# liuzhenboo/Stereo-Visual-Odometry

Measured on AMD Instinct MI355X. Metric: stereo frames/sec on KITTI-00 1241x376; LK-kernel achieved HBM GB/s vs peak, higher is better.
Workload: dtype u8; 1 GPU; S0 synthetic KITTI-like stereo sequence 1241x376 (config #2 stand-in), FAST+LK track_mode LK_stereof2f_pnp, batched frame pairs (256 per step, 4 distinct chunks cycled), frames resident in HBM for `value`; `m1` (--full) = host-resident frames, H2D included; pairs_ok_last_step=256, parallelism=1 GPU

## Files before the change

### include/svo_abi.h

```cpp
#ifndef SVO_ABI_H
#define SVO_ABI_H

#include <stdint.h>

#ifdef __cplusplus
extern "C" {
#endif

#define SVO_ABI_VERSION 9

#define SVO_OK                 0
#define SVO_ERR_ARG           -1
#define SVO_ERR_HIP           -2
#define SVO_ERR_NOMEM         -3
#define SVO_ERR_STATE         -4
#define SVO_FAIL_FEW_KEYPOINTS 1
#define SVO_FAIL_FEW_TRACKS    2
#define SVO_FAIL_INLIER_RATIO  3
#define SVO_FAIL_ROTATION_GATE 4
#define SVO_FAIL_TRANSL_GATE   5
#define SVO_FAIL_CAPACITY      6

#define SVO_MEM_HOST   0
#define SVO_MEM_DEVICE 1

typedef struct svo_ctx svo_ctx;

typedef struct { float x, y; } svo_pt2f;
typedef struct { float x, y, z; } svo_pt3f;
typedef struct {
    float x, y, size, angle, response;
    int32_t octave, class_id;
} svo_keypoint;

typedef struct {
    int32_t width, height;
    int32_t max_keypoints;
    int32_t max_batch;
    int32_t num_slots;
    int32_t fast_threshold;
    int32_t num_features_tracking;
    int32_t iterations;
    float   reproj_err;
    float   confidence;
    double  feature_match_error;
    double  inlier_rate;
    double  min_move2, max_move2;
    double  P1[12], P2[12];
    int32_t track_mode;
    int32_t orb_nfeatures;
    float   orb_scale_factor;
    int32_t orb_nlevels;
    int32_t orb_ini_th, orb_min_th;
    int32_t lk_accum;
    int32_t fast_keep_strongest;
} svo_config;

#define SVO_MODE_LK  0
#define SVO_MODE_ORB 1
#define SVO_LK_ACCUM_EXACT 0
#define SVO_LK_ACCUM_SSE2  1
#define SVO_LK_ACCUM_SIMD128 2
#define SVO_LK_ACCUM_SSE2_LEGACY 3

typedef struct {
    double rvec[3], tvec[3], R[9];
    int32_t n_inliers, ransac_iters, best_iter, lm_iters, ok, _pad;
} svo_pnp_result;

typedef struct {
    int32_t ok;
    int32_t fail_stage;
    int32_t n_prev_kps, n_cur_kps, n_tracked, n_inliers;
    int32_t ransac_iters, lm_iters;
    double  rvec[3], tvec[3], R[9];
    double  T_rel_inv[16];
    double  pose[16];
} svo_step_result;

int         svo_abi_version(void);
int         svo_config_bytes(void);
void        svo_default_config(svo_config *cfg, int width, int height);
int         svo_device_count(int *n);
int         svo_create(const svo_config *cfg, int device, svo_ctx **out);
void        svo_destroy(svo_ctx *ctx);
const char *svo_last_error(const svo_ctx *ctx);
int         svo_set_stream(svo_ctx *ctx, void *hip_stream);
int         svo_sync(svo_ctx *ctx);
int         svo_wait_stream(svo_ctx *ctx, void *hip_stream);
int         svo_signal_stream(svo_ctx *ctx, void *hip_stream);
int         svo_signal_stream_inputs(svo_ctx *ctx, void *hip_stream);
int         svo_num_levels(const svo_ctx *ctx);


int svo_fast_detect(svo_ctx *ctx, const uint8_t *img, int pitch, int mem, int threshold,
                    int nonmax, svo_keypoint *out, int cap, int *n_out);

int svo_build_pyramid(svo_ctx *ctx, int slot, const uint8_t *img, int pitch, int mem);
int svo_read_pyramid_level(svo_ctx *ctx, int slot, int level, uint8_t *out, int out_pitch, int mem,
                           int *w, int *h);

int svo_lk_track(svo_ctx *ctx, int slot_prev, int slot_next, const svo_pt2f *prev_pts, int n,
                 svo_pt2f *next_pts, uint8_t *status, int mem);

int svo_circular_match(svo_ctx *ctx, int slot_prevL, int slot_prevR, int slot_curL, int slot_curR,
                       const svo_pt2f *t1_left, int n, svo_pt2f *out_t1_left,
                       svo_pt2f *out_t1_right, svo_pt2f *out_t2_right, svo_pt2f *out_t2_left,
                       int *m_out, int mem);

int svo_triangulate(svo_ctx *ctx, const double P1[12], const double P2[12], const svo_pt2f *x1,
                    const svo_pt2f *x2, int n, svo_pt3f *out, int mem);

int svo_pnp_ransac(svo_ctx *ctx, const svo_pt3f *obj, const svo_pt2f *img, int n, const double K[9],
                   int iterations, float reproj_err, double confidence, svo_pnp_result *res,
                   uint8_t *inlier_mask, int mem);

int svo_orb_extract(svo_ctx *ctx, const uint8_t *img, int pitch, int mem, svo_keypoint *kps, uint8_t *desc,
                    int cap, int *n_out, int *per_level);
int svo_orb_read_level(svo_ctx *ctx, int level, uint8_t *out, int *w, int *h);
int svo_orb_read_candidates(svo_ctx *ctx, int level, float *out4, int cap, int *n_out);

int svo_match_hamming(svo_ctx *ctx, const uint8_t *query, int nq, const uint8_t *train, int nt, int32_t *train_idx,
                      float *distance, int mem);


int svo_add_frame(svo_ctx *ctx, const uint8_t *left, const uint8_t *right, int pitch, int mem,
                  svo_step_result *res);
int svo_reset(svo_ctx *ctx);
int svo_get_pose(svo_ctx *ctx, double pose[16]);
int svo_set_pose(svo_ctx *ctx, const double pose[16]);

int svo_track_batch(svo_ctx *ctx, const uint8_t *left_frames, const uint8_t *right_frames,
                    int pitch, int64_t frame_stride, int n_frames, const double *pose0,
                    svo_step_result *results, int results_mem);

int svo_set_overlap(svo_ctx *ctx, int on);
int svo_wait_results(svo_ctx *ctx);

int svo_host_alloc(svo_ctx *ctx, size_t bytes, void **out);
int svo_host_free(svo_ctx *ctx, void *p);
int svo_upload_frames(svo_ctx *ctx, int buf, const uint8_t *left_frames, const uint8_t *right_frames,
                      int pitch, int64_t frame_stride, int n_frames);
int svo_upload_frames_at(svo_ctx *ctx, int buf, int first_slot, const uint8_t *left_frames, const uint8_t *right_frames,
                         int pitch, int64_t frame_stride, int n_frames);
int svo_wait_upload(svo_ctx *ctx, int buf);
int svo_track_uploaded(svo_ctx *ctx, int buf, int n_frames, const double *pose0,
                       svo_step_result *results, int results_mem);
#define SVO_CONTINUE_CHAIN       1
#define SVO_CONTINUE_CARRY_FRAME 2
int svo_track_uploaded_async(svo_ctx *ctx, int buf, int n_frames, const double *pose0, int continue_chain);
int svo_collect_results(svo_ctx *ctx, svo_step_result *results, int n_pairs);
int svo_results_ready(svo_ctx *ctx, int *n_pairs);

int svo_get_frame_keypoints(svo_ctx *ctx, int side, svo_keypoint *kps, uint8_t *descriptors, int cap, int *n_out);
int svo_get_last_tracks(svo_ctx *ctx, svo_pt2f *t1_left, svo_pt2f *t1_right, svo_pt2f *t2_right,
                        svo_pt2f *t2_left, uint8_t *inlier, int cap, int *n_out);
int svo_get_batch_tracks(svo_ctx *ctx, int pair, svo_pt2f *t1_left, svo_pt2f *t1_right, svo_pt2f *t2_right,
                         svo_pt2f *t2_left, uint8_t *inlier, int cap, int *n_out);

int svo_streams_create(svo_ctx *ctx, int n_streams);
int svo_streams_count(const svo_ctx *ctx, int *n_streams);
int svo_streams_step(svo_ctx *ctx, const int32_t *stream_ids, int m, const uint8_t *left_frames,
                     const uint8_t *right_frames, int pitch, int64_t frame_stride, int mem,
                     svo_step_result *results, int results_mem);
int svo_streams_reset(svo_ctx *ctx, int stream_id);
int svo_streams_get_pose(svo_ctx *ctx, int stream_id, double pose[16]);
int svo_streams_set_pose(svo_ctx *ctx, int stream_id, const double pose[16]);
int svo_streams_get_tracks(svo_ctx *ctx, int item, svo_pt2f *t1_left, svo_pt2f *t1_right, svo_pt2f *t2_right,
                           svo_pt2f *t2_left, uint8_t *inlier, int cap, int *n_out);

#define SVO_INTERP_NEAREST 0
#define SVO_INTERP_LINEAR  1
int svo_scale_projection(const double P[12], double inv_x, double inv_y, int interp, double P_out[12]);
int svo_resize(svo_ctx *ctx, const uint8_t *src, int sw, int sh, int spitch, int64_t sstride,
               uint8_t *dst, int dw, int dh, int dpitch, int64_t dstride, int n_frames,
               int interp, double fx, double fy, int mem);
int svo_ingest_create(svo_ctx *ctx, int src_width, int src_height, int interp, double fx, double fy);
int svo_ingest_info(const svo_ctx *ctx, int *src_width, int *src_height, int *interp, double *inv_x, double *inv_y);
int svo_ingest_add_frame(svo_ctx *ctx, const uint8_t *left, const uint8_t *right, int pitch, int mem, svo_step_result *res);
int svo_ingest_track_batch(svo_ctx *ctx, const uint8_t *lefts, const uint8_t *rights, int pitch, int64_t frame_stride,
                           int n_frames, const double *pose0, svo_step_result *results, int results_mem);
int svo_ingest_streams_step(svo_ctx *ctx, const int32_t *stream_ids, int m, const uint8_t *lefts, const uint8_t *rights,
                            int pitch, int64_t frame_stride, int mem, svo_step_result *results, int results_mem);
// ... 57 lines not shown
```

### stereo-visual-odometry_amd/binding.py

```python
import ctypes as C
import os
import subprocess

import numpy as np

_HERE = os.path.dirname(os.path.abspath(__file__))
_LIB = None

MEM_HOST, MEM_DEVICE = 0, 1

KP_DTYPE = np.dtype([("x", "<f4"), ("y", "<f4"), ("size", "<f4"), ("angle", "<f4"),
                     ("response", "<f4"), ("octave", "<i4"), ("class_id", "<i4")])


class SvoError(RuntimeError):
    pass


class Config(C.Structure):
    _fields_ = [("width", C.c_int32), ("height", C.c_int32), ("max_keypoints", C.c_int32),
                ("max_batch", C.c_int32), ("num_slots", C.c_int32), ("fast_threshold", C.c_int32),
                ("num_features_tracking", C.c_int32), ("iterations", C.c_int32),
                ("reproj_err", C.c_float), ("confidence", C.c_float),
                ("feature_match_error", C.c_double), ("inlier_rate", C.c_double),
# ... 57 lines not shown
    return library_path()


def load_library():
    global _LIB
    if _LIB is not None:
        return _LIB
    path = library_path()
    if not os.path.exists(path):
        raise SvoError(f"{path} is missing: run __graft_entry__.build() (hipcc) first; "
                       "this package has no CPU fallback")
    lib = C.CDLL(path)
    if lib.svo_config_bytes() != C.sizeof(Config):
        raise SvoError(f"{path}: svo_config is {lib.svo_config_bytes()} bytes, this binding's Config {C.sizeof(Config)} "
                       "(stale build? run __graft_entry__.build())")
    lib.svo_last_error.restype = C.c_char_p
    lib.svo_last_error.argtypes = [C.c_void_p]
    lib.svo_create.argtypes = [C.POINTER(Config), C.c_int, C.POINTER(C.c_void_p)]
    lib.svo_destroy.argtypes = [C.c_void_p]
    lib.svo_destroy.restype = None
    lib.svo_default_config.argtypes = [C.POINTER(Config), C.c_int, C.c_int]
    lib.svo_default_config.restype = None
    lib.svo_track_batch.argtypes = [C.c_void_p, C.c_void_p, C.c_void_p, C.c_int, C.c_int64, C.c_int,
                                    C.c_void_p, C.c_void_p, C.c_int]
    lib.svo_get_frame_keypoints.argtypes = [C.c_void_p, C.c_int, C.c_void_p, C.c_void_p, C.c_int, C.POINTER(C.c_int)]
    lib.svo_get_last_tracks.argtypes = [C.c_void_p] + [C.c_void_p] * 5 + [C.c_int, C.POINTER(C.c_int)]
    lib.svo_get_batch_tracks.argtypes = [C.c_void_p, C.c_int] + [C.c_void_p] * 5 + [C.c_int, C.POINTER(C.c_int)]
    lib.svo_chain_relative.argtypes = [C.c_void_p, C.c_void_p, C.c_void_p, C.c_int, C.c_void_p, C.c_void_p, C.c_int]
    lib.svo_host_alloc.argtypes = [C.c_void_p, C.c_size_t, C.POINTER(C.c_void_p)]
    lib.svo_host_free.argtypes = [C.c_void_p, C.c_void_p]
    lib.svo_upload_frames.argtypes = [C.c_void_p, C.c_int, C.c_void_p, C.c_void_p, C.c_int, C.c_int64, C.c_int]
    lib.svo_upload_frames_at.argtypes = [C.c_void_p, C.c_int, C.c_int, C.c_void_p, C.c_void_p, C.c_int, C.c_int64, C.c_int]
    lib.svo_wait_stream.argtypes = [C.c_void_p, C.c_void_p]
    lib.svo_signal_stream.argtypes = [C.c_void_p, C.c_void_p]
    lib.svo_signal_stream_inputs.argtypes = [C.c_void_p, C.c_void_p]
    lib.svo_wait_upload.argtypes = [C.c_void_p, C.c_int]
    lib.svo_track_uploaded.argtypes = [C.c_void_p, C.c_int, C.c_int, C.c_void_p, C.c_void_p, C.c_int]
    lib.svo_track_uploaded_async.argtypes = [C.c_void_p, C.c_int, C.c_int, C.c_void_p, C.c_int]
    lib.svo_collect_results.argtypes = [C.c_void_p, C.c_void_p, C.c_int]
    lib.svo_results_ready.argtypes = [C.c_void_p, C.POINTER(C.c_int)]
    lib.svo_set_pose.argtypes = [C.c_void_p, C.c_void_p]
    lib.svo_streams_create.argtypes = [C.c_void_p, C.c_int]
    lib.svo_streams_count.argtypes = [C.c_void_p, C.POINTER(C.c_int)]
    lib.svo_streams_step.argtypes = [C.c_void_p, C.c_void_p, C.c_int, C.c_void_p, C.c_void_p, C.c_int, C.c_int64, C.c_int,
                                     C.c_void_p, C.c_int]
    lib.svo_streams_reset.argtypes = [C.c_void_p, C.c_int]
    lib.svo_streams_get_pose.argtypes = [C.c_void_p, C.c_int, C.c_void_p]
    lib.svo_streams_set_pose.argtypes = [C.c_void_p, C.c_int, C.c_void_p]
    lib.svo_streams_get_tracks.argtypes = [C.c_void_p, C.c_int] + [C.c_void_p] * 5 + [C.c_int, C.POINTER(C.c_int)]
    lib.svo_scale_projection.argtypes = [C.c_void_p, C.c_double, C.c_double, C.c_int, C.c_void_p]
    lib.svo_resize.argtypes = [C.c_void_p, C.c_void_p, C.c_int, C.c_int, C.c_int, C.c_int64,
                               C.c_void_p, C.c_int, C.c_int, C.c_int, C.c_int64, C.c_int, C.c_int, C.c_double, C.c_double, C.c_int]
    lib.svo_ingest_create.argtypes = [C.c_void_p, C.c_int, C.c_int, C.c_int, C.c_double, C.c_double]
    lib.svo_ingest_info.argtypes = [C.c_void_p, C.POINTER(C.c_int), C.POINTER(C.c_int), C.POINTER(C.c_int),
                                    C.POINTER(C.c_double), C.POINTER(C.c_double)]
    lib.svo_ingest_add_frame.argtypes = [C.c_void_p, C.c_void_p, C.c_void_p, C.c_int, C.c_int, C.c_void_p]
    lib.svo_ingest_track_batch.argtypes = lib.svo_track_batch.argtypes
    lib.svo_ingest_streams_step.argtypes = lib.svo_streams_step.argtypes
    lib.svo_ingest_upload_frames_at.argtypes = lib.svo_upload_frames_at.argtypes
    lib.svo_set_fast_buckets.argtypes = [C.c_void_p, C.c_int, C.c_int, C.c_int]
    lib.svo_get_fast_buckets.argtypes = [C.c_void_p, C.POINTER(C.c_int), C.POINTER(C.c_int), C.POINTER(C.c_int)]
    lib.svo_bucket_corners.argtypes = [C.c_void_p, C.c_void_p, C.c_int, C.c_int, C.c_int, C.c_int, C.c_int, C.c_int,
                                       C.c_void_p, C.c_int, C.c_void_p, C.c_int]
    lib.svo_set_lk_detector.argtypes = [C.c_void_p, C.c_int, C.c_int, C.c_double, C.c_double]
    lib.svo_get_lk_detector.argtypes = [C.c_void_p, C.POINTER(C.c_int), C.POINTER(C.c_int), C.POINTER(C.c_double),
                                        C.POINTER(C.c_double)]
    lib.svo_min_eigen_map.argtypes = [C.c_void_p, C.c_void_p, C.c_int, C.c_int, C.c_int, C.c_int, C.c_void_p, C.c_int]
    lib.svo_gftt_detect.argtypes = [C.c_void_p, C.c_void_p, C.c_int, C.c_int, C.c_int, C.c_int, C.c_int, C.c_double, C.c_double,
                                    C.c_void_p, C.c_void_p, C.c_int, C.c_void_p]
    lib.svo_set_pose_refine.argtypes = [C.c_void_p, C.c_int, C.c_int, C.c_int, C.c_double, C.c_int]
    lib.svo_get_pose_refine.argtypes = [C.c_void_p, C.POINTER(C.c_int), C.POINTER(C.c_int), C.POINTER(C.c_int),
                                        C.POINTER(C.c_double), C.POINTER(C.c_int)]
    lib.svo_refine_pose.argtypes = [C.c_void_p, C.c_void_p, C.c_void_p, C.c_void_p, C.c_int, C.c_void_p, C.c_void_p, C.c_void_p,
                                    C.c_void_p, C.POINTER(RefineResult), C.c_void_p, C.c_int]
    lib.svo_get_refine_result.argtypes = [C.c_void_p, C.c_int, C.POINTER(RefineResult), C.c_void_p, C.c_int, C.POINTER(C.c_int)]
    lib.svo_set_orb_matcher.argtypes = [C.c_void_p, C.c_int, C.c_int, C.c_int, C.c_double, C.c_double, C.c_double]
    lib.svo_get_orb_matcher.argtypes = [C.c_void_p, C.POINTER(C.c_int), C.POINTER(C.c_int), C.POINTER(C.c_int),
                                        C.POINTER(C.c_double), C.POINTER(C.c_double), C.POINTER(C.c_double)]
    lib.svo_orb_stereo_frame.argtypes = [C.c_void_p, C.c_void_p, C.c_void_p, C.c_int, C.c_int, C.c_int, C.c_void_p, C.c_void_p,
                                         C.c_void_p, C.c_int, C.POINTER(C.c_int)]
    lib.svo_orb_track_frames.argtypes = [C.c_void_p, C.c_int, C.c_int, C.c_void_p, C.c_void_p, C.c_void_p, C.c_void_p, C.c_void_p,
                                         C.c_int, C.POINTER(C.c_int)]
    lib.svo_get_frame_stereo.argtypes = [C.c_void_p, C.c_void_p, C.c_void_p, C.c_int, C.POINTER(C.c_int)]
    _LIB = lib
    return lib


def _interp(interp):
    if isinstance(interp, str):
        if interp not in ("nearest", "linear"):
            raise ValueError(f"interp must be 'nearest' or 'linear', not {interp!r}")
        return INTERP_LINEAR if interp == "linear" else INTERP_NEAREST
    return int(interp)


def scale_projection(P, inv_x, inv_y, interp="nearest"):
    P = np.ascontiguousarray(P, np.float64).reshape(12)
    out = np.zeros(12)
    rc = load_library().svo_scale_projection(C.c_void_p(P.ctypes.data), float(inv_x), float(inv_y), _interp(interp),
                                             C.c_void_p(out.ctypes.data))
    if rc != 0:
        raise SvoError(f"svo_scale_projection failed ({rc}): inv must be in (0, 1], interp nearest or linear")
    return out.reshape(3, 4)


def device_count():
    n = C.c_int(0)
    load_library().svo_device_count(C.byref(n))
    return n.value


def default_config(width, height, **overrides):
    cfg = Config()
    load_library().svo_default_config(C.byref(cfg), int(width), int(height))
    for k, v in overrides.items():
        if k in ("P1", "P2"):
            arr = getattr(cfg, k)
            for i, x in enumerate(np.asarray(v, np.float64).reshape(12)):
                arr[i] = float(x)
        else:
            setattr(cfg, k, v)
    return cfg


def _ptr(a):
    if a is None:
        return None, MEM_HOST
    if isinstance(a, np.ndarray):
        assert a.flags["C_CONTIGUOUS"]
        return C.c_void_p(a.ctypes.data), MEM_HOST
    assert a.is_contiguous()
    return C.c_void_p(a.data_ptr()), (MEM_DEVICE if a.is_cuda else MEM_HOST)


def _pose_ptr(pose0):
    if pose0 is None:
        return None
    return np.ascontiguousarray(pose0, np.float64).reshape(16).ctypes.data_as(C.c_void_p)


def _records(n, results):
    if results is None:
        out = np.zeros(n, dtype=STEP_DTYPE)
        return out, C.c_void_p(out.ctypes.data), MEM_HOST
    return results, C.c_void_p(results.data_ptr()), MEM_DEVICE


class Context:

    def __init__(self, width, height, device=0, **cfg_overrides):
        self.lib = load_library()
        self.cfg = default_config(width, height, **cfg_overrides)
        h = C.c_void_p()
        rc = self.lib.svo_create(C.byref(self.cfg), int(device), C.byref(h))
        if rc != 0:
            raise SvoError(f"svo_create failed with {rc} (no usable HIP device?) -- there is no CPU fallback")
        self.h = h
        self.width, self.height = int(width), int(height)

    def close(self):
        if getattr(self, "h", None):
            self.lib.svo_destroy(self.h)
            self.h = None

    def __del__(self):
        try:
# ... 5 lines not shown
        if rc < 0 or (rc > 0 and not allow_soft):
            raise SvoError(f"svo call failed ({rc}): {self.lib.svo_last_error(self.h).decode()}")
        return rc

    def sync(self):
        self._check(self.lib.svo_sync(self.h))

    def set_stream(self, stream_handle):
        self._check(self.lib.svo_set_stream(self.h, C.c_void_p(stream_handle)))
        self._stream_handle = int(stream_handle or 0)

    def wait_stream(self, stream_handle):
        self._check(self.lib.svo_wait_stream(self.h, C.c_void_p(stream_handle)))

    def signal_stream(self, stream_handle):
        self._check(self.lib.svo_signal_stream(self.h, C.c_void_p(stream_handle)))

    def signal_stream_inputs(self, stream_handle):
        self._check(self.lib.svo_signal_stream_inputs(self.h, C.c_void_p(stream_handle)))

    def _order_in(self, t):
        import torch
        other = torch.cuda.current_stream(t.device).cuda_stream
        if other and other == getattr(self, "_stream_handle", 0):
            return False
        self.wait_stream(other)
        return True

    def _order_out(self, t):
        import torch
        other = torch.cuda.current_stream(t.device).cuda_stream
        if other and other == getattr(self, "_stream_handle", 0):
            return
        self.signal_stream(other)

    @property
    def num_levels(self):
        return self.lib.svo_num_levels(self.h)

    def set_overlap(self, on=True):
        self._check(self.lib.svo_set_overlap(self.h, int(on)))

    def wait_results(self):
        self._check(self.lib.svo_wait_results(self.h))

    def enable_timing(self, on=True):
        self._check(self.lib.svo_enable_timing(self.h, int(on)))

    def get_timing(self):
        names = (C.c_char_p * 64)()
        ms = (C.c_float * 64)()
        n = self.lib.svo_get_timing(self.h, names, ms, 64)
        return [(names[i].decode(), float(ms[i])) for i in range(n)]

    def _img(self, img, shape=None):
        shape = shape or (self.height, self.width)
        assert tuple(img.shape) == tuple(shape), (tuple(img.shape), shape)
        if isinstance(img, np.ndarray):
            assert img.dtype == np.uint8 and img.strides[1] == 1
            return C.c_void_p(img.ctypes.data), int(img.strides[0]), MEM_HOST
        assert img.element_size() == 1 and img.stride(1) == 1
        return C.c_void_p(img.data_ptr()), int(img.stride(0)), (MEM_DEVICE if img.is_cuda else MEM_HOST)

    def fast_detect(self, img, threshold=20, nonmax=True, cap=None):
        cap = cap or self.cfg.max_keypoints
        p, pitch, mem = self._img(img)
        out = np.zeros(cap, dtype=KP_DTYPE)
        n = C.c_int(0)
        self._check(self.lib.svo_fast_detect(self.h, p, pitch, mem, int(threshold), int(bool(nonmax)),
                                             C.c_void_p(out.ctypes.data), cap, C.byref(n)))
        return out[:n.value].copy()

    def build_pyramid(self, slot, img):
        p, pitch, mem = self._img(img)
        self._check(self.lib.svo_build_pyramid(self.h, int(slot), p, pitch, mem))

    def read_pyramid_level(self, slot, level):
        w, h = C.c_int(0), C.c_int(0)
        self._check(self.lib.svo_read_pyramid_level(self.h, slot, level, None, 0, MEM_HOST,
                                                    C.byref(w), C.byref(h)))
        out = np.zeros((h.value, w.value), np.uint8)
        self._check(self.lib.svo_read_pyramid_level(self.h, slot, level, C.c_void_p(out.ctypes.data),
                                                    w.value, MEM_HOST, C.byref(w), C.byref(h)))
        return out

    def lk_track(self, slot_prev, slot_next, pts):
        if isinstance(pts, np.ndarray):
            pts = np.ascontiguousarray(pts, np.float32).reshape(-1, 2)
            n = pts.shape[0]
            out = np.zeros((n, 2), np.float32)
            st = np.zeros(n, np.uint8)
        else:
            import torch
            n = pts.shape[0]
            out = torch.zeros((n, 2), dtype=torch.float32, device=pts.device)
            st = torch.zeros(n, dtype=torch.uint8, device=pts.device)
            self._order_in(st)
        pi, mem = _ptr(pts)
        po, _ = _ptr(out)
        ps, _ = _ptr(st)
        self._check(self.lib.svo_lk_track(self.h, slot_prev, slot_next, pi, n, po, ps, mem))
        if mem == MEM_DEVICE:
            self._order_out(st)
        return out, st

    def circular_match(self, slots, t1_left):
        if isinstance(t1_left, np.ndarray):
            t1_left = np.ascontiguousarray(t1_left, np.float32).reshape(-1, 2)
            n = t1_left.shape[0]
            outs = [np.zeros((max(n, 1), 2), np.float32) for _ in range(4)]
        else:
            import torch
            n = t1_left.shape[0]
            outs = [torch.zeros((max(n, 1), 2), dtype=torch.float32, device=t1_left.device) for _ in range(4)]
            self._order_in(outs[0])
        pi, mem = _ptr(t1_left)
        m = C.c_int(0)
        self._check(self.lib.svo_circular_match(self.h, *[int(s) for s in slots], pi, n,
                                                *[_ptr(o)[0] for o in outs], C.byref(m), mem))
        return [o[:m.value] for o in outs]

    def triangulate(self, P1, P2, x1, x2):
        P1 = np.ascontiguousarray(P1, np.float64).reshape(12)
        P2 = np.ascontiguousarray(P2, np.float64).reshape(12)
        if isinstance(x1, np.ndarray):
            x1 = np.ascontiguousarray(x1, np.float32).reshape(-1, 2)
            x2 = np.ascontiguousarray(x2, np.float32).reshape(-1, 2)
            out = np.zeros((x1.shape[0], 3), np.float32)
        else:
            import torch
            out = torch.zeros((x1.shape[0], 3), dtype=torch.float32, device=x1.device)
            self._order_in(out)
        p1, mem = _ptr(x1)
        p2, _ = _ptr(x2)
        self._check(self.lib.svo_triangulate(self.h, C.c_void_p(P1.ctypes.data), C.c_void_p(P2.ctypes.data),
                                             p1, p2, x1.shape[0], _ptr(out)[0], mem))
        if mem == MEM_DEVICE:
            self._order_out(out)
        return out

    def pnp_ransac(self, obj, img, K, iterations=500, reproj_err=0.5, confidence=0.99):
        K = np.ascontiguousarray(K, np.float64).reshape(9)
        if isinstance(obj, np.ndarray):
            obj = np.ascontiguousarray(obj, np.float32).reshape(-1, 3)
            img = np.ascontiguousarray(img, np.float32).reshape(-1, 2)
            mask = np.zeros(max(obj.shape[0], 1), np.uint8)
        else:
            import torch
            mask = torch.zeros(max(obj.shape[0], 1), dtype=torch.uint8, device=obj.device)
            self._order_in(mask)
        n = obj.shape[0]
        res = PnPResult()
        po, mem = _ptr(obj)
        conf = float(np.float32(confidence))
        self._check(self.lib.svo_pnp_ransac(self.h, po, _ptr(img)[0], n, C.c_void_p(K.ctypes.data),
                                            int(iterations), C.c_float(reproj_err), C.c_double(conf),
                                            C.byref(res), _ptr(mask)[0], mem))
        if mem == MEM_DEVICE:
            self._order_out(mask)
            mask = mask.cpu().numpy()
        return dict(ok=res.ok, rvec=np.array(res.rvec), tvec=np.array(res.tvec),
                    R=np.array(res.R).reshape(3, 3), n_inliers=res.n_inliers,
                    ransac_iters=res.ransac_iters, best_iter=res.best_iter, lm_iters=res.lm_iters,
                    mask=np.asarray(mask[:n]).copy())

    def set_pose_refine(self, mode, rounds=4, iters=10, sigma_px=1.0, min_inliers=6):
# ... 490 lines not shown
```

### stereo-visual-odometry_amd/csrc/pyramid.hip

```cpp
#include "svo_device.h"
#include "svo_kernels.h"

namespace svo {

__device__ __forceinline__ const uint8_t *src_image(const PyrArgs &a, int b)
{
    if (a.img2) return ((b & 1) ? a.img2 : a.img) + (int64_t)(b >> 1) * a.img_stride;
    return a.img + (int64_t)b * a.img_stride;
}

__global__ __launch_bounds__(256) void pyr_copy0_kernel(PyrArgs a)
{
    const int b = blockIdx.z, y = blockIdx.y * blockDim.y + threadIdx.y;
    const int w = a.g.w[0];
    if (y >= a.g.h[0]) return;
    const uint8_t *src = src_image(a, b) + (int64_t)y * a.pitch;
    uint8_t *dst = a.slots + (int64_t)b * a.slot_stride + a.g.origin[0] + (int64_t)y * a.g.pitch[0];
    const int x = (blockIdx.x * blockDim.x + threadIdx.x) * 16;
    if (x >= w) return;
    if (x + 16 <= w && ((uintptr_t)(src + x) & 15) == 0) {
        *(uint4 *)(dst + x) = *(const uint4 *)(src + x);
    } else {
        for (int q = 0; q < 16 && x + q < w; q++) dst[x + q] = src[x + q];
    }
}

constexpr int kBorderRows = 16;
constexpr int kFrameRowsPerWg = 4, kSidePasses = 4;
__host__ __device__ inline int border_top_groups() { return 2 * kPad / kFrameRowsPerWg; }
__host__ __device__ inline int border_side_groups(int h) { return (h + kBorderRows * kSidePasses - 1) / (kBorderRows * kSidePasses); }
__global__ __launch_bounds__(256) void pyr_border_kernel(PyrArgs a, int l)
{
    const int b = blockIdx.y;
    const int w = a.g.w[l], h = a.g.h[l], pitch = a.g.pitch[l];
    uint8_t *lvl = a.slots + (int64_t)b * a.slot_stride + a.g.origin[l];
    if ((int)blockIdx.x < border_top_groups()) {
        for (int q = 0; q < kFrameRowsPerWg; q++) {
            const int gidx = blockIdx.x * kFrameRowsPerWg + q;
            const int py = gidx < kPad ? gidx - kPad : h + (gidx - kPad);
            const uint8_t *src = lvl + (int64_t)refl101(py, h) * pitch;
            uint8_t *dst = lvl + (int64_t)py * pitch;
            for (int px = ((int)threadIdx.x << 2) - kPad; px < w + kPad; px += 1024) {
                uint32_t v = 0;
                if (px >= 0 && px + 4 <= w) v = *(const uint32_t *)(src + px);
                else {
#pragma unroll
                    for (int k = 0; k < 4; k++) v |= (uint32_t)src[refl101(min(px + k, w + kPad - 1), w)] << (8 * k);
                }
                if (px + 4 <= w + kPad) *(uint32_t *)(dst + px) = v;
                else for (int k = 0; px + k < w + kPad; k++) dst[px + k] = (uint8_t)(v >> (8 * k));
            }
        }
        return;
    }
    const int sgroup = blockIdx.x - border_top_groups();
    if (w >= 2 * kPad) {
        static_assert(kBorderRows == 16 && kPad == 32, "256 threads = 16 rows x 16 dwords");
        typedef uint32_t u32_unaligned __attribute__((aligned(1)));
        const int k = threadIdx.x & 15, r = threadIdx.x >> 4;
        const int px = k < 8 ? -kPad + 4 * k : w + 4 * (k - 8);
        const int c0 = k < 8 ? kPad - 3 - 4 * k : w - 5 - 4 * (k - 8);
        for (int q = 0; q < kSidePasses; q++) {
            const int py = (sgroup * kSidePasses + q) * kBorderRows + r;
            if (py >= h) return;
            uint8_t *row = lvl + (int64_t)py * pitch;
            const uint32_t v = *(const u32_unaligned *)(row + c0);
            *(u32_unaligned *)(row + px) = __builtin_amdgcn_perm(0u, v, 0x00010203u);
        }
    } else {
        const int t = threadIdx.x & 63;
        const int px = t < kPad ? t - kPad : w + (t - kPad);
        const int sx = refl101(px, w);
        for (int q = 0; q < kSidePasses; q++)
            for (int r = threadIdx.x >> 6; r < kBorderRows; r += 4) {
                const int py = (sgroup * kSidePasses + q) * kBorderRows + r;
                if (py >= h) return;
                uint8_t *row = lvl + (int64_t)py * pitch;
                row[px] = row[sx];
            }
    }
}

__global__ __launch_bounds__(256) void pyr_down_kernel(PyrArgs a, int l)
{
    const int b = blockIdx.z, y = blockIdx.y * blockDim.y + threadIdx.y;
    const int w = a.g.w[l];
    if (y >= a.g.h[l]) return;
    const int sp = a.g.pitch[l - 1];
    uint8_t *slot = a.slots + (int64_t)b * a.slot_stride;
    const uint8_t *src = slot + a.g.origin[l - 1];
    uint8_t *dst = slot + a.g.origin[l] + (int64_t)y * a.g.pitch[l];
    const int x0 = (blockIdx.x * blockDim.x + threadIdx.x) * 4;
    if (x0 >= w) return;
    int acc[4] = {0, 0, 0, 0};
#pragma unroll
    for (int r = 0; r < 5; r++) {
        const uint32_t *row = (const uint32_t *)(src + (int64_t)(2 * y + r - 2) * sp + 2 * x0 - 4);
        const uint32_t d0 = row[0], d1 = row[1], d2 = row[2], d3 = row[3];
        int s[16];
#pragma unroll
        for (int j = 0; j < 4; j++) {
            s[j] = (d0 >> (8 * j)) & 255; s[4 + j] = (d1 >> (8 * j)) & 255;
            s[8 + j] = (d2 >> (8 * j)) & 255; s[12 + j] = (d3 >> (8 * j)) & 255;
        }
        const int wv = (r == 2) ? 6 : ((r == 1 || r == 3) ? 4 : 1);
#pragma unroll
        for (int q = 0; q < 4; q++) {
            const int c = 4 + 2 * q;
            const int hs = s[c] * 6 + (s[c - 1] + s[c + 1]) * 4 + s[c - 2] + s[c + 2];
            acc[q] += hs * wv;
        }
    }
    uint32_t out = 0;
#pragma unroll
    for (int q = 0; q < 4; q++) out |= (uint32_t)((acc[q] + 128) >> 8) << (8 * q);
    if (x0 + 4 <= w) *(uint32_t *)(dst + x0) = out;
    else for (int q = 0; x0 + q < w; q++) dst[x0 + q] = (uint8_t)(out >> (8 * q));
}

__global__ __launch_bounds__(256) void pyr_read_level_kernel(PyrGeom g, const uint8_t *slot, int l,
                                                              uint8_t *out, int out_pitch)
{
    int x = blockIdx.x * 256 + threadIdx.x, y = blockIdx.y;
    if (x >= g.w[l]) return;
    out[(int64_t)y * out_pitch + x] = slot[g.origin[l] + (int64_t)y * g.pitch[l] + x];
}

void launch_pyramid(const PyrArgs &a, int batch, hipStream_t st)
{
    dim3 blk(256, 1, 1);
    auto shape = [](int lanes_per_row, int rows, dim3 &grid, dim3 &block, int batch) {
        const int bx = lanes_per_row < 256 ? lanes_per_row : 256, by = 256 / bx;
        block = dim3(bx, by, 1);
        grid = dim3((lanes_per_row + bx - 1) / bx, (rows + by - 1) / by, batch);
    };
    {
        dim3 g, bk;
        shape((a.g.w[0] + 15) / 16, a.g.h[0], g, bk, batch);
        hipLaunchKernelGGL(pyr_copy0_kernel, g, bk, 0, st, a);
    }
    for (int l = 0; l < a.g.nlevels; l++) {
        if (l > 0) {
            dim3 g, bk;
            shape((a.g.w[l] + 3) / 4, a.g.h[l], g, bk, batch);
            hipLaunchKernelGGL(pyr_down_kernel, g, bk, 0, st, a, l);
        }
        dim3 gb(border_top_groups() + border_side_groups(a.g.h[l]), batch, 1);
        hipLaunchKernelGGL(pyr_border_kernel, gb, blk, 0, st, a, l);
    }
}

void launch_pyr_read_level(const PyrGeom &g, const uint8_t *slot, int l, uint8_t *out, int out_pitch,
                           hipStream_t st)
{
    dim3 grid((g.w[l] + 255) / 256, g.h[l], 1), blk(256, 1, 1);
    hipLaunchKernelGGL(pyr_read_level_kernel, grid, blk, 0, st, g, slot, l, out, out_pitch);
}

}
```

### stereo-visual-odometry_amd/csrc/svo_abi.hip

```cpp
#include <cmath>
#include <cstdio>
#include <cstring>
#include <ctime>
#include <new>
#include <vector>
#include "svo_ctx.h"

using namespace svo;

static int align_up(int v, int a) { return (v + a - 1) / a * a; }

namespace svo {
int dev_alloc_raw(svo_ctx *ctx, void **out, size_t bytes)
{
    *out = nullptr;
    if (bytes == 0) bytes = 1;
    if (ctx->arena.planning) {
        ctx->arena.plan.emplace_back(out, ctx->arena.planned);
        ctx->arena.planned += (bytes + 255) / 256 * 256;
        return SVO_OK;
    }
    SVO_HIP(hipMalloc(out, bytes));
    ctx->arena.extra.push_back(*out);
    return SVO_OK;
// ... 382 lines not shown
    return svo::stage_host_image(ctx, img, pitch, stage_idx, dptr, dpitch);
}

extern "C" int svo_fast_detect(svo_ctx *ctx, const uint8_t *img, int pitch, int mem, int threshold,
                               int nonmax, svo_keypoint *out, int cap, int *n_out)
{
    if (!ctx) return SVO_ERR_ARG;
    SVO_ARG(out && n_out && cap >= 0, "null output");
    SVO_HIP(hipSetDevice(ctx->device));
    const uint8_t *d; int dp;
    int rc = resolve_image(ctx, img, pitch, mem, 0, &d, &dp);
    if (rc) return rc;
    FastArgs a{};
    a.img = d; a.pitch = dp; a.img_stride = 0;
    a.w = ctx->cfg.width; a.h = ctx->cfg.height;
    a.thr = threshold < 0 ? 0 : (threshold > 255 ? 255 : threshold);
    a.nms = nonmax != 0;
    a.score = ctx->score; a.spitch = ctx->spitch; a.score_stride = ctx->score_stride;
    a.rowcount = ctx->rowcount; a.rowcount_stride = ctx->rowcount_stride;
    a.kp_xy = ctx->kp_xy; a.kp_resp = ctx->kp_resp; a.kp_stride = ctx->cfg.max_keypoints;
    a.n_out = ctx->kp_n; a.cap = ctx->cfg.max_keypoints;
    launch_fast(a, 1, ctx->stream);
    SVO_HIP(hipGetLastError());
    int *h_n = (int *)ctx->h_pinned;
    SVO_HIP(hipMemcpyAsync(h_n, ctx->kp_n, sizeof(int), hipMemcpyDeviceToHost, ctx->stream));
    SVO_HIP(hipStreamSynchronize(ctx->stream));
    int n = *h_n;
    *n_out = n;
    if (n > ctx->cfg.max_keypoints) { ctx->err = "FAST: keypoints exceed max_keypoints"; return SVO_ERR_ARG; }
    if (n > cap) { ctx->err = "FAST: keypoints exceed caller capacity"; return SVO_ERR_ARG; }
    if (n == 0) return SVO_OK;
    float2 *h_xy = (float2 *)((char *)ctx->h_pinned + 256);
    float *h_r = (float *)(h_xy + ctx->cfg.max_keypoints);
    SVO_HIP(hipMemcpyAsync(h_xy, ctx->kp_xy, sizeof(float2) * n, hipMemcpyDeviceToHost, ctx->stream));
    SVO_HIP(hipMemcpyAsync(h_r, ctx->kp_resp, sizeof(float) * n, hipMemcpyDeviceToHost, ctx->stream));
    SVO_HIP(hipStreamSynchronize(ctx->stream));
    for (int i = 0; i < n; i++) {
        out[i].x = h_xy[i].x; out[i].y = h_xy[i].y; out[i].size = 7.f; out[i].angle = -1.f;
        out[i].response = h_r[i]; out[i].octave = 0; out[i].class_id = -1;
    }
    return SVO_OK;
}

extern "C" int svo_build_pyramid(svo_ctx *ctx, int slot, const uint8_t *img, int pitch, int mem)
{
    if (!ctx) return SVO_ERR_ARG;
    SVO_ARG(slot >= 0 && slot < ctx->cfg.num_slots, "slot out of range");
    SVO_HIP(hipSetDevice(ctx->device));
    const uint8_t *d; int dp;
    int rc = resolve_image(ctx, img, pitch, mem, 0, &d, &dp);
    if (rc) return rc;
    PyrArgs a{};
    a.g = ctx->geom; a.img = d; a.pitch = dp; a.img_stride = 0;
    a.slots = ctx->slots + (size_t)slot * ctx->geom.slot_bytes; a.slot_stride = 0;
    launch_pyramid(a, 1, ctx->stream);
    SVO_HIP(hipGetLastError());
    if (mem == SVO_MEM_HOST) SVO_HIP(hipStreamSynchronize(ctx->stream));
    ctx->slot_built[slot] = 1;
    return SVO_OK;
}

extern "C" int svo_read_pyramid_level(svo_ctx *ctx, int slot, int level, uint8_t *out, int out_pitch,
                                      int mem, int *w, int *h)
{
    if (!ctx) return SVO_ERR_ARG;
    SVO_ARG(slot >= 0 && slot < ctx->cfg.num_slots, "slot out of range");
    SVO_ARG(level >= 0 && level < ctx->geom.nlevels, "level out of range");
    if (!ctx->slot_built[slot]) { ctx->err = "pyramid slot not built"; return SVO_ERR_STATE; }
    const int lw = ctx->geom.w[level], lh = ctx->geom.h[level];
    if (w) *w = lw;
    if (h) *h = lh;
    if (!out) return SVO_OK;
    SVO_ARG(out_pitch >= lw, "out_pitch < level width");
    SVO_HIP(hipSetDevice(ctx->device));
    const uint8_t *s = ctx->slots + (size_t)slot * ctx->geom.slot_bytes;
    if (mem == SVO_MEM_DEVICE) {
        launch_pyr_read_level(ctx->geom, s, level, out, out_pitch, ctx->stream);
        SVO_HIP(hipGetLastError());
        return SVO_OK;
    }
    SVO_HIP(hipMemcpy2DAsync(out, out_pitch, s + ctx->geom.origin[level], ctx->geom.pitch[level], lw, lh,
                             hipMemcpyDeviceToHost, ctx->stream));
    SVO_HIP(hipStreamSynchronize(ctx->stream));
    return SVO_OK;
}

template <typename T>
static int to_device(svo_ctx *ctx, const T *src, T *scratch, int n, int mem, const T **d)
{
    if (mem == SVO_MEM_DEVICE) { *d = src; return SVO_OK; }
    SVO_HIP(hipMemcpyAsync(scratch, src, sizeof(T) * (size_t)n, hipMemcpyHostToDevice, ctx->stream));
    *d = scratch;
    return SVO_OK;
}

static void fill_lk_common(svo_ctx *ctx, LkArgs &a, int n)
{
    a.g = ctx->geom;
    a.slot_stride = 0;
    a.pts_stride = 0;
    a.n_pts = nullptr; a.n_fixed = n; a.cap = n;
    a.match_err = ctx->cfg.feature_match_error;
    a.accum = ctx->cfg.lk_accum;
}

extern "C" int svo_lk_track(svo_ctx *ctx, int slot_prev, int slot_next, const svo_pt2f *prev_pts, int n,
                            svo_pt2f *next_pts, uint8_t *status, int mem)
{
    if (!ctx) return SVO_ERR_ARG;
    SVO_ARG(slot_prev >= 0 && slot_prev < ctx->cfg.num_slots && slot_next >= 0 &&
            slot_next < ctx->cfg.num_slots, "slot out of range");
    SVO_ARG(n >= 0 && n <= ctx->cfg.max_keypoints, "n exceeds max_keypoints");
    SVO_ARG(mem == SVO_MEM_HOST || mem == SVO_MEM_DEVICE, "bad mem");
    if (!ctx->slot_built[slot_prev] || !ctx->slot_built[slot_next]) { ctx->err = "pyramid slot not built"; return SVO_ERR_STATE; }
    if (n == 0) return SVO_OK;
    SVO_ARG(prev_pts && next_pts && status, "null pointer");
    SVO_HIP(hipSetDevice(ctx->device));
    const float2 *d_in;
    int rc = to_device<float2>(ctx, (const float2 *)prev_pts, ctx->pts_in, n, mem, &d_in);
    if (rc) return rc;
    LkArgs a{};
    fill_lk_common(ctx, a, n);
    a.ncalls = 1;
    a.prev[0] = ctx->slots + (size_t)slot_prev * ctx->geom.slot_bytes;
    a.next[0] = ctx->slots + (size_t)slot_next * ctx->geom.slot_bytes;
    a.pts_in = d_in;
    a.pts_out[0] = mem == SVO_MEM_DEVICE ? (float2 *)next_pts : ctx->pts_out[0];
    a.status[0] = mem == SVO_MEM_DEVICE ? status : ctx->status[0];
    launch_lk(a, 1, n, ctx->stream);
    SVO_HIP(hipGetLastError());
    if (mem == SVO_MEM_HOST) {
        SVO_HIP(hipMemcpyAsync(next_pts, ctx->pts_out[0], sizeof(float2) * (size_t)n, hipMemcpyDeviceToHost, ctx->stream));
        SVO_HIP(hipMemcpyAsync(status, ctx->status[0], (size_t)n, hipMemcpyDeviceToHost, ctx->stream));
        SVO_HIP(hipStreamSynchronize(ctx->stream));
    }
    return SVO_OK;
}

extern "C" int svo_circular_match(svo_ctx *ctx, int slot_prevL, int slot_prevR, int slot_curL, int slot_curR,
                                  const svo_pt2f *t1_left, int n, svo_pt2f *out_t1_left,
                                  svo_pt2f *out_t1_right, svo_pt2f *out_t2_right, svo_pt2f *out_t2_left,
                                  int *m_out, int mem)
{
    if (!ctx) return SVO_ERR_ARG;
    const int sl[4] = {slot_prevL, slot_prevR, slot_curL, slot_curR};
    for (int i = 0; i < 4; i++) {
        SVO_ARG(sl[i] >= 0 && sl[i] < ctx->cfg.num_slots, "slot out of range");
        if (!ctx->slot_built[sl[i]]) { ctx->err = "pyramid slot not built"; return SVO_ERR_STATE; }
    }
    SVO_ARG(n >= 0 && n <= ctx->cfg.max_keypoints, "n exceeds max_keypoints");
    SVO_ARG(mem == SVO_MEM_HOST || mem == SVO_MEM_DEVICE, "bad mem");
    SVO_ARG(m_out != nullptr, "null m_out");
    if (svo_wait_results(ctx) != SVO_OK) return SVO_ERR_HIP;
    *m_out = 0;
    if (n == 0) return SVO_OK;
    SVO_ARG(t1_left && out_t1_left && out_t1_right && out_t2_right && out_t2_left, "null pointer");
    SVO_HIP(hipSetDevice(ctx->device));
    const float2 *d_in;
    int rc = to_device<float2>(ctx, (const float2 *)t1_left, ctx->pts_in, n, mem, &d_in);
    if (rc) return rc;
    auto S = [&](int s) { return ctx->slots + (size_t)s * ctx->geom.slot_bytes; };
    LkArgs a{};
    fill_lk_common(ctx, a, n);
    a.ncalls = 4;
    a.prev[0] = S(slot_prevL); a.next[0] = S(slot_prevR);
    a.prev[1] = S(slot_prevR); a.next[1] = S(slot_curR);
// ... 1045 lines not shown
```

Baseline: 19600 stereo pairs/s.

## Fuse level-0 border reflection into pyramid copy kernel

The level-0 copy kernel now writes the reflected top and bottom border rows while copying interior rows, and adds extra lanes per row that write the mirrored left and right side borders. The separate border kernel launch for level 0 is then skipped. This removes one kernel launch and a re-read of the freshly written level-0 image. In exchange some threads do extra stores and unaligned accesses. A padded-pyramid read API is added so the borders can be validated.

Result: no change. 19660 stereo pairs/s (median of 6 runs) (+0.3%).

```diff
diff --git a/include/svo_abi.h b/include/svo_abi.h
--- a/include/svo_abi.h
+++ b/include/svo_abi.h
@@ -99,6 +99,8 @@
 int svo_build_pyramid(svo_ctx *ctx, int slot, const uint8_t *img, int pitch, int mem);
 int svo_read_pyramid_level(svo_ctx *ctx, int slot, int level, uint8_t *out, int out_pitch, int mem,
                            int *w, int *h);
+int svo_read_pyramid_padded(svo_ctx *ctx, int slot, int level, uint8_t *out, int out_pitch, int mem,
+                            int *w, int *h, int *pad, int frame_slots);
 
 int svo_lk_track(svo_ctx *ctx, int slot_prev, int slot_next, const svo_pt2f *prev_pts, int n,
                  svo_pt2f *next_pts, uint8_t *status, int mem);
diff --git a/stereo-visual-odometry_amd/binding.py b/stereo-visual-odometry_amd/binding.py
--- a/stereo-visual-odometry_amd/binding.py
+++ b/stereo-visual-odometry_amd/binding.py
@@ -163,6 +163,8 @@
     lib.svo_orb_track_frames.argtypes = [C.c_void_p, C.c_int, C.c_int, C.c_void_p, C.c_void_p, C.c_void_p, C.c_void_p, C.c_void_p,
                                          C.c_int, C.POINTER(C.c_int)]
     lib.svo_get_frame_stereo.argtypes = [C.c_void_p, C.c_void_p, C.c_void_p, C.c_int, C.POINTER(C.c_int)]
+    lib.svo_read_pyramid_padded.argtypes = [C.c_void_p, C.c_int, C.c_int, C.c_void_p, C.c_int, C.c_int, C.POINTER(C.c_int),
+                                            C.POINTER(C.c_int), C.POINTER(C.c_int), C.c_int]
     _LIB = lib
     return lib
 
@@ -334,6 +336,15 @@
         out = np.zeros((h.value, w.value), np.uint8)
         self._check(self.lib.svo_read_pyramid_level(self.h, slot, level, C.c_void_p(out.ctypes.data),
                                                     w.value, MEM_HOST, C.byref(w), C.byref(h)))
+        return out
+
+    def read_pyramid_padded(self, slot, level, frame_slots=False):
+        w, h, pad = C.c_int(0), C.c_int(0), C.c_int(0)
+        self._check(self.lib.svo_read_pyramid_padded(self.h, int(slot), int(level), None, 0, MEM_HOST, C.byref(w), C.byref(h),
+                                                     C.byref(pad), int(bool(frame_slots))))
+        out = np.zeros((h.value + 2 * pad.value, w.value + 2 * pad.value), np.uint8)
+        self._check(self.lib.svo_read_pyramid_padded(self.h, int(slot), int(level), C.c_void_p(out.ctypes.data), out.shape[1],
+                                                     MEM_HOST, None, None, None, int(bool(frame_slots))))
         return out
 
     def lk_track(self, slot_prev, slot_next, pts):
diff --git a/stereo-visual-odometry_amd/csrc/pyramid.hip b/stereo-visual-odometry_amd/csrc/pyramid.hip
--- a/stereo-visual-odometry_amd/csrc/pyramid.hip
+++ b/stereo-visual-odometry_amd/csrc/pyramid.hip
@@ -9,19 +9,59 @@
     return a.img + (int64_t)b * a.img_stride;
 }
 
+#ifndef SVO_PYR_FUSED_FRAMES
+#define SVO_PYR_FUSED_FRAMES 1
+#endif
+__host__ __device__ inline bool frame_fused(int w, int h) { return SVO_PYR_FUSED_FRAMES && w >= 2 * kPad && h > kPad; }
+constexpr int kCopySideLanes = 4;
+typedef uint32_t u32_unaligned __attribute__((aligned(1)));
+__device__ __forceinline__ uint32_t byte_reverse(uint32_t v) { return __builtin_amdgcn_perm(0u, v, 0x00010203u); }
+
+struct FrameRows { int up, dn; };
+__device__ __forceinline__ FrameRows frame_rows(int y, int h, bool fused)
+{
+    FrameRows r;
+    r.up = (fused && y >= 1 && y <= kPad) ? -2 * y : 0;
+    r.dn = (fused && y >= h - 1 - kPad && y <= h - 2) ? 2 * (h - 1 - y) : 0;
+    return r;
+}
+template <typename F>
+__device__ __forceinline__ void store_rows(uint8_t *row, int pitch, FrameRows r, F store)
+{
+    store(row);
+    if (r.up) store(row + (int64_t)r.up * pitch);
+    if (r.dn) store(row + (int64_t)r.dn * pitch);
+}
+
 __global__ __launch_bounds__(256) void pyr_copy0_kernel(PyrArgs a)
 {
     const int b = blockIdx.z, y = blockIdx.y * blockDim.y + threadIdx.y;
-    const int w = a.g.w[0];
-    if (y >= a.g.h[0]) return;
+    const int w = a.g.w[0], h = a.g.h[0], pitch = a.g.pitch[0];
+    if (y >= h) return;
+    const bool fused = frame_fused(w, h);
+    const FrameRows fr = frame_rows(y, h, fused);
     const uint8_t *src = src_image(a, b) + (int64_t)y * a.pitch;
-    uint8_t *dst = a.slots + (int64_t)b * a.slot_stride + a.g.origin[0] + (int64_t)y * a.g.pitch[0];
-    const int x = (blockIdx.x * blockDim.x + threadIdx.x) * 16;
-    if (x >= w) return;
-    if (x + 16 <= w && ((uintptr_t)(src + x) & 15) == 0) {
-        *(uint4 *)(dst + x) = *(const uint4 *)(src + x);
+    uint8_t *dst = a.slots + (int64_t)b * a.slot_stride + a.g.origin[0] + (int64_t)y * pitch;
+    const int lane = blockIdx.x * blockDim.x + threadIdx.x, n_int = (w + 15) / 16;
+    const int j = lane - n_int, t = j & 1;
+    const bool side = j >= 0;
+    if (side && (!fused || j >= kCopySideLanes)) return;
+    const int x = side ? (j < 2 ? kPad - 15 - 16 * t : w - 17 - 16 * t) : lane * 16;
+    const int px = side ? (j < 2 ? -kPad + 16 * t : w + 16 * t) : x;
+    if (side || (x + 16 <= w && ((uintptr_t)(src + x) & 15) == 0)) {
+        const u32_unaligned *s4 = (const u32_unaligned *)(src + x);
+        const uint32_t d0 = s4[0], d1 = s4[1], d2 = s4[2], d3 = s4[3];
+        const uint32_t v0 = side ? byte_reverse(d3) : d0, v1 = side ? byte_reverse(d2) : d1;
+        const uint32_t v2 = side ? byte_reverse(d1) : d2, v3 = side ? byte_reverse(d0) : d3;
+        store_rows(dst, pitch, fr, [&](uint8_t *row) {
+            u32_unaligned *o = (u32_unaligned *)(row + px);
+            o[0] = v0; o[1] = v1; o[2] = v2; o[3] = v3;
+        });
     } else {
-        for (int q = 0; q < 16 && x + q < w; q++) dst[x + q] = src[x + q];
+        for (int q = 0; q < 16 && x + q < w; q++) {
+            const uint8_t v = src[x + q];
+            store_rows(dst, pitch, fr, [&](uint8_t *row) { row[x + q] = v; });
+        }
     }
 }
 
@@ -56,7 +96,6 @@
     const int sgroup = blockIdx.x - border_top_groups();
     if (w >= 2 * kPad) {
         static_assert(kBorderRows == 16 && kPad == 32, "256 threads = 16 rows x 16 dwords");
-        typedef uint32_t u32_unaligned __attribute__((aligned(1)));
         const int k = threadIdx.x & 15, r = threadIdx.x >> 4;
         const int px = k < 8 ? -kPad + 4 * k : w + 4 * (k - 8);
         const int c0 = k < 8 ? kPad - 3 - 4 * k : w - 5 - 4 * (k - 8);
@@ -65,7 +104,7 @@
             if (py >= h) return;
             uint8_t *row = lvl + (int64_t)py * pitch;
             const uint32_t v = *(const u32_unaligned *)(row + c0);
-            *(u32_unaligned *)(row + px) = __builtin_amdgcn_perm(0u, v, 0x00010203u);
+            *(u32_unaligned *)(row + px) = byte_reverse(v);
         }
     } else {
         const int t = threadIdx.x & 63;
@@ -134,9 +173,10 @@
         block = dim3(bx, by, 1);
         grid = dim3((lanes_per_row + bx - 1) / bx, (rows + by - 1) / by, batch);
     };
+    const bool fused0 = frame_fused(a.g.w[0], a.g.h[0]);
     {
         dim3 g, bk;
-        shape((a.g.w[0] + 15) / 16, a.g.h[0], g, bk, batch);
+        shape((a.g.w[0] + 15) / 16 + (fused0 ? kCopySideLanes : 0), a.g.h[0], g, bk, batch);
         hipLaunchKernelGGL(pyr_copy0_kernel, g, bk, 0, st, a);
     }
     for (int l = 0; l < a.g.nlevels; l++) {
@@ -145,6 +185,7 @@
             shape((a.g.w[l] + 3) / 4, a.g.h[l], g, bk, batch);
             hipLaunchKernelGGL(pyr_down_kernel, g, bk, 0, st, a, l);
         }
+        if (l == 0 && fused0) continue;
         dim3 gb(border_top_groups() + border_side_groups(a.g.h[l]), batch, 1);
         hipLaunchKernelGGL(pyr_border_kernel, gb, blk, 0, st, a, l);
     }
diff --git a/stereo-visual-odometry_amd/csrc/svo_abi.hip b/stereo-visual-odometry_amd/csrc/svo_abi.hip
--- a/stereo-visual-odometry_amd/csrc/svo_abi.hip
+++ b/stereo-visual-odometry_amd/csrc/svo_abi.hip
@@ -488,6 +488,35 @@
     SVO_HIP(hipMemcpy2DAsync(out, out_pitch, s + ctx->geom.origin[level], ctx->geom.pitch[level], lw, lh,
                              hipMemcpyDeviceToHost, ctx->stream));
     SVO_HIP(hipStreamSynchronize(ctx->stream));
+    return SVO_OK;
+}
+
+extern "C" int svo_read_pyramid_padded(svo_ctx *ctx, int slot, int level, uint8_t *out, int out_pitch,
+                                       int mem, int *w, int *h, int *pad, int frame_slots)
+{
+    if (!ctx) return SVO_ERR_ARG;
+    SVO_ARG(level >= 0 && level < ctx->geom.nlevels, "level out of range");
+    const uint8_t *s;
+    if (frame_slots) {
+        SVO_ARG(ctx->cfg.track_mode == SVO_MODE_LK, "frame slots hold LK pyramids in LK mode only");
+        SVO_ARG(slot >= 0 && slot < 2 * ctx->n_img, "image slot out of range");
+        s = ctx->bslots + (size_t)slot * ctx->geom.slot_bytes;
+    } else {
+        SVO_ARG(slot >= 0 && slot < ctx->cfg.num_slots, "slot out of range");
+        if (!ctx->slot_built[slot]) { ctx->err = "pyramid slot not built"; return SVO_ERR_STATE; }
+        s = ctx->slots + (size_t)slot * ctx->geom.slot_bytes;
+    }
+    const int pw = ctx->geom.w[level] + 2 * kPad, ph = ctx->geom.h[level] + 2 * kPad, pitch = ctx->geom.pitch[level];
+    if (w) *w = ctx->geom.w[level];
+    if (h) *h = ctx->geom.h[level];
+    if (pad) *pad = kPad;
+    if (!out) return SVO_OK;
+    SVO_ARG(out_pitch >= pw, "out_pitch < padded level width");
+    SVO_ARG(mem == SVO_MEM_HOST || mem == SVO_MEM_DEVICE, "mem must be SVO_MEM_HOST or SVO_MEM_DEVICE");
+    SVO_HIP(hipSetDevice(ctx->device));
+    SVO_HIP(hipMemcpy2DAsync(out, out_pitch, s + ctx->geom.origin[level] - (int64_t)kPad * pitch - kPad, pitch, pw, ph,
+                             mem == SVO_MEM_HOST ? hipMemcpyDeviceToHost : hipMemcpyDeviceToDevice, ctx->stream));
+    if (mem == SVO_MEM_HOST) SVO_HIP(hipStreamSynchronize(ctx->stream));
     return SVO_OK;
 }
 
```
